# tritonmedia/beholder

Hardware: AMD Instinct MI355X
Metric: metric_events_ingested_per_sec (higher is better)
Workload: dtype protobuf-events (no tensor compute); 1 GPU; model=beholder telemetry consumer (status+progress handlers, index.js:62-155), global_batch=65536, parallelism=dp1 x 1 consumer proc/rank (BASELINE: single process per consumer)

## Files before the change

### beholder_amd/ops/csrc/py_handlers.cpp

```cpp
#include <cstdlib>
#include <string>
#include <vector>

#include "native_api.hpp"
#include "py_common.hpp"

namespace beholder {
PyTypeObject* h1_response_type();
PyObject* h1_response_status(PyObject* resp);
}
#include "gil_clock.hpp"
#include "ring.hpp"

namespace beholder {

bool text_js_str_append(std::string& out, PyObject* v);
bool text_query_pair_append(std::string& out, PyObject* k, PyObject* v, bool* first, bool rfc3986);
PyObject* pg_pool_execute_c(PyObject* nets, PyObject* sql, PyObject* params, PyObject* spread_at, PyObject* size);
PyObject* h1_call_new(PyObject* client, PyObject* method, PyObject* url, PyObject* params, PyObject* timeout,
                      bool front);
bool is_native_logger(PyObject* logger);
bool logcore_emit(PyObject* logger, bool native, long lvl, PyObject* const* args, Py_ssize_t nargs);
bool sink_stats_record(PyObject* stats, PyObject* status, double seconds);
bool is_sink_stats(PyObject* o);
// ... 248 lines not shown
bool catch_and_warn(HandlersObject* hs, PyObject* text) {
  if (!PyErr_ExceptionMatches(PyExc_Exception)) return false;
  PyObject *et, *ev, *tb;
  PyErr_Fetch(&et, &ev, &tb);
  PyErr_NormalizeException(&et, &ev, &tb);
  Py_XDECREF(tb);
  Py_XDECREF(et);
  if (ev) PyException_SetTraceback(ev, Py_None);
  PyObject* msg = PyObject_CallOneArg(hs->err_message, ev ? ev : Py_None);
  Py_XDECREF(ev);
  if (!msg) return false;
  PyObject* args[2] = {text, msg};
  bool ok = log_line(hs, 40, args, 2);
  Py_DECREF(msg);
  return ok;
}

PySendResult finish_ack(CallObject* c, PyObject** result) {
  c->done = 1;
  PyObject* r = Py_TYPE(c->rmsg) == &DeliveryType ? delivery_ack_c(c->rmsg)
                                                   : PyObject_CallMethodNoArgs(c->rmsg, s_ack);
  if (!r) return PYGEN_ERROR;
  *result = r;
  return PYGEN_RETURN;
}

PySendResult fail(CallObject* c) {
  c->done = 1;
  return PYGEN_ERROR;
}

bool raise_to_lower_case(HandlersObject* hs) {
  PyErr_SetObject(hs->js_type_error, hs->x[X_ERR_TO_LOWER]);
  return false;
}

PyObject* const* const kStoreKeys[3] = {&s_pool, &s_select, &s_update};
PyObject* const* const kPoolKeys[4] = {&s_native_pick, &s_conns, &s_spread_at, &s_size};

int pg_execute(CallObject* c, PyObject* store, PyObject* sql_name, PyObject* params, PyObject** out) {
  HandlersObject* hs = c->hs;
  if (reinterpret_cast<PyObject*>(Py_TYPE(store)) != hs->pg_cls) return 2;
  PyObject** dp = _PyObject_GetDictPtr(store);
  PyObject* sd = dp ? *dp : nullptr;
  if (!sd || !PyDict_CheckExact(sd)) return 2;
  if (!hs->store_view.refresh(sd, kStoreKeys)) return -1;
  PyObject* pool = hs->store_view.v[0];
  PyObject* sql = sql_name == s_select ? hs->store_view.v[1] : sql_name == s_update ? hs->store_view.v[2] : nullptr;
  if (!sql && pool && sql_name != s_select && sql_name != s_update) {
    sql = PyDict_GetItemWithError(sd, sql_name);
    if (!sql && PyErr_Occurred()) return -1;
  }
  if (!pool || pool == Py_None || !sql) return 2;
  PyObject** pdp = reinterpret_cast<PyObject*>(Py_TYPE(pool)) == hs->pool_cls ? _PyObject_GetDictPtr(pool) : nullptr;
  PyObject* pd = pdp ? *pdp : nullptr;
  if (pd && PyDict_CheckExact(pd) && !hs->pool_view.refresh(pd, kPoolKeys)) return -1;
  PyObject* pick = pd && PyDict_CheckExact(pd) ? hs->pool_view.v[0] : nullptr;
  if (pick && pick == hs->pick_fn) {
    PyObject* conns = hs->pool_view.v[1];
    PyObject* spread = hs->pool_view.v[2];
    PyObject* size = hs->pool_view.v[3];
    if (conns && spread && size && PyList_CheckExact(conns)) {
      Py_INCREF(conns);
      PyObject* f = pg_pool_execute_c(conns, sql, params, spread, size);
      Py_DECREF(conns);
      if (!f) return -1;
      if (f != Py_None) return await_start(c, f, out);
      Py_DECREF(f);
    }
  }
  PyObject* args[3] = {pool, sql, params};
  Py_INCREF(pool);
  PyObject* aw = PyObject_VectorcallMethod(s_execute, args, 3, nullptr);
  Py_DECREF(pool);
  if (!aw) return -1;
  return await_start(c, aw, out);
}

void untrack_row(PyObject* t) {
  if (!PyObject_GC_IsTracked(t) || Py_TYPE(t)->tp_dictoffset != 0) return;
  for (Py_ssize_t i = 0, n = PyTuple_GET_SIZE(t); i < n; ++i) {
    PyObject* v = PyTuple_GET_ITEM(t, i);
    if (PyObject_IS_GC(v) && PyObject_GC_IsTracked(v)) return;
  }
  PyObject_GC_UnTrack(t);
}

PyObject* pg_media(CallObject* c, PyObject* res) {
  HandlersObject* hs = c->hs;
  PyObject* rows = PyTuple_Check(res) && PyTuple_GET_SIZE(res) == 2 ? PyTuple_GET_ITEM(res, 0) : nullptr;
  if (!rows || !PyList_Check(rows)) {
    Py_DECREF(res);
    PyErr_SetString(PyExc_TypeError, "unexpected Postgres result");
    return nullptr;
  }
  if (PyList_GET_SIZE(rows) == 0) {
    Py_DECREF(res);
    PyErr_SetObject(hs->not_found, c->media_id);
    return nullptr;
  }
  PyObject* r = PyList_GET_ITEM(rows, 0);
  Py_INCREF(r);
  Py_DECREF(res);
  bool fast = hs->media_cls && PyTuple_CheckExact(r) && PyTuple_GET_SIZE(r) == 10;
  for (Py_ssize_t i = 0; fast && i < 10; ++i) {
    PyObject* v = PyTuple_GET_ITEM(r, i);
    bool is_int_col = i == 2 || i == 4 || i == 5 || i == 7 || i == 9;
    if (v == Py_None || (is_int_col && !PyLong_CheckExact(v))) fast = false;
  }
  PyObject* m;
  if (fast) {
    PyObject* args = PyTuple_Pack(1, r);
    m = args ? PyTuple_Type.tp_new(reinterpret_cast<PyTypeObject*>(hs->media_cls), args, nullptr) : nullptr;
    Py_XDECREF(args);
    if (m) untrack_row(m);
  } else {
    m = PyObject_CallOneArg(hs->row_to_media, r);
  }
  Py_DECREF(r);
  return m;
}

}

void untrack_atomic_row(PyObject* t) { untrack_row(t); }

namespace {

int get_media(CallObject* c, PyObject** out) {
  HandlersObject* hs = c->hs;
  PyObject* store = hattr(hs, s_store);
  if (!store) return -1;
  if (reinterpret_cast<PyObject*>(Py_TYPE(store)) == hs->memory_cls) {
    PyObject** dp = _PyObject_GetDictPtr(store);
    PyObject* sd = dp ? *dp : nullptr;
    PyObject* rows = sd ? PyDict_GetItemWithError(sd, s_rows) : nullptr;
    PyObject* calls = rows ? PyDict_GetItemWithError(sd, s_get_calls) : nullptr;
    if (calls && PyDict_CheckExact(rows)) {
      PyObject* n = PyNumber_Add(calls, hs->one);
      if (!n) return -1;
      int rc = PyDict_SetItem(sd, s_get_calls, n);
      Py_DECREF(n);
      if (rc < 0) return -1;
      PyObject* m = PyDict_GetItemWithError(rows, c->media_id);
      if (!m) {
        if (!PyErr_Occurred()) PyErr_SetObject(hs->not_found, c->media_id);
        return -1;
      }
      Py_INCREF(m);
      *out = m;
      return 1;
    }
    if (PyErr_Occurred()) return -1;
  }
  PyObject* params = PyTuple_Pack(1, c->media_id);
  if (!params) return -1;
  int k = pg_execute(c, store, s_select, params, out);
  Py_DECREF(params);
  if (k != 2) {
    if (k == 0) c->pg_get = 1;
    if (k == 1 && !(*out = pg_media(c, *out))) return -1;
    return k;
  }
  PyObject* get = hattr(hs, s_get_nowait);
  if (!get) return -1;
  if (get != Py_None) {
    PyObject* m = PyObject_CallOneArg(get, c->media_id);
    if (!m) return -1;
    *out = m;
    return 1;
  }
  PyObject* aw = PyObject_CallMethodOneArg(store, s_get_by_id, c->media_id);
  if (!aw) return -1;
  return await_start(c, aw, out);
}

int update_inline(CallObject* c) {
  HandlersObject* hs = c->hs;
  PyObject* store = hattr(hs, s_store);
  if (!store) return -1;
  if (reinterpret_cast<PyObject*>(Py_TYPE(store)) != hs->memory_cls || !hs->media_cls ||
      !PyLong_CheckExact(c->status))
    return 0;
  PyObject** dp = _PyObject_GetDictPtr(store);
  PyObject* sd = dp ? *dp : nullptr;
  PyObject* rows = sd ? PyDict_GetItemWithError(sd, s_rows) : nullptr;
  PyObject* calls = rows ? PyDict_GetItemWithError(sd, s_update_calls) : nullptr;
  if (!calls || !PyDict_CheckExact(rows)) return PyErr_Occurred() ? -1 : 0;
  PyObject* n = PyNumber_Add(calls, hs->one);
  if (!n) return -1;
  int rc = PyDict_SetItem(sd, s_update_calls, n);
  Py_DECREF(n);
  if (rc < 0) return -1;
  PyObject* m = PyDict_GetItemWithError(rows, c->media_id);
  if (!m) return PyErr_Occurred() ? -1 : 1;
  if (reinterpret_cast<PyObject*>(Py_TYPE(m)) != hs->media_cls) {
    PyObject* kw = Py_BuildValue("{s:O}", "status", c->status);
    PyObject* meth = kw ? PyObject_GetAttrString(m, "_replace") : nullptr;
    PyObject* nm = meth ? PyObject_Call(meth, PyTuple_New(0), kw) : nullptr;
    Py_XDECREF(meth);
    Py_XDECREF(kw);
    if (!nm) return -1;
    rc = PyDict_SetItem(rows, c->media_id, nm);
    Py_DECREF(nm);
    return rc < 0 ? -1 : 1;
  }
  Py_ssize_t len = PyTuple_GET_SIZE(m);
  PyObject* items = PyTuple_New(len);
  if (!items) return -1;
  for (Py_ssize_t i = 0; i < len; ++i) {
    PyObject* v = i == hs->ix_m[2] ? c->status : PyTuple_GET_ITEM(m, i);
    Py_INCREF(v);
    PyTuple_SET_ITEM(items, i, v);
  }
  PyObject* args = PyTuple_Pack(1, items);
  Py_DECREF(items);
  if (!args) return -1;
  PyObject* nm = PyTuple_Type.tp_new(reinterpret_cast<PyTypeObject*>(hs->media_cls), args, nullptr);
  Py_DECREF(args);
  if (!nm) return -1;
  untrack_row(nm);
  rc = PyDict_SetItem(rows, c->media_id, nm);
  Py_DECREF(nm);
  return rc < 0 ? -1 : 1;
}

bool record_stats(PyObject* stats, PyObject* status, double seconds) {
  if (is_sink_stats(stats)) return sink_stats_record(stats, status, seconds);
  PyObject* sec = PyFloat_FromDouble(seconds);
  if (!sec) return false;
  PyObject* r = PyObject_CallMethodObjArgs(stats, s_record, status, sec, nullptr);
  Py_DECREF(sec);
  if (!r) return false;
  Py_DECREF(r);
  return true;
}

void count_request(CallObject* c) {
  if (c->nreq < 255) ++c->nreq;
}

PyObject* const* const kHttpKeys[2] = {&s_native_record, &s_native_call};

PyObject* http_request(CallObject* c, PyObject* http, PyObject* method, PyObject* url, PyObject* params,
                       PyObject* timeout) {
  HandlersObject* hs = c->hs;
  const bool front = c->nreq > 0;
  count_request(c);
  PyObject** dp = _PyObject_GetDictPtr(http);
  PyObject* hd = dp && *dp && PyDict_CheckExact(*dp) ? *dp : nullptr;
  if (hd && !hs->http_view.refresh(hd, kHttpKeys)) return nullptr;
  PyObject* rec = hd ? hs->http_view.v[0] : nullptr;
  if (rec && PyCapsule_CheckExact(rec) && PyCapsule_IsValid(rec, kSinkHookName)) {
    const SinkHook* hook = static_cast<const SinkHook*>(PyCapsule_GetPointer(rec, kSinkHookName));
    PyObject* self = static_cast<PyObject*>(PyCapsule_GetContext(rec));
    if (!hook || !self || hook->abi != kSinkHookAbi) {
      if (!PyErr_Occurred()) PyErr_SetString(PyExc_RuntimeError, "native_record: incompatible sink hook");
      return nullptr;
    }
    Py_INCREF(rec);
    PyObject* r = hook->request(self, method, url, params ? params : Py_None);
    Py_DECREF(rec);
    return r;
  }
  PyObject* cur = hd ? hs->http_view.v[1] : nullptr;
  if (cur && cur == hs->h1_fast_fn) {
    PyObject* call = h1_call_new(http, method, url, params ? params : Py_None, timeout, front);
    if (call != Py_None) return call;
    Py_DECREF(call);
  } else if (PyErr_Occurred()) {
    return nullptr;
  }
  if (params) {
    PyObject* args[5] = {http, method, url, params, timeout};
    return PyObject_VectorcallMethod(s_request, args, 3, kw_params_timeout);
  }
  PyObject* args[4] = {http, method, url, timeout};
  return PyObject_VectorcallMethod(s_request, args, 3, kw_timeout);
}

PyObject* request_finish(CallObject* c, PyObject* value) {
  if (!c->req_native) return value;
  c->req_native = 0;
  PyObject* stats = c->req_stats;
  c->req_stats = nullptr;
  double dt = double(gil_mono_ns() - c->req_t0) * 1e-9;
  if (!value) {
    if (stats) {
      PyObject *et, *ev, *tb;
      PyErr_Fetch(&et, &ev, &tb);
      if (record_stats(stats, Py_None, dt)) {
        PyErr_Restore(et, ev, tb);
      } else {
        Py_XDECREF(et);
        Py_XDECREF(ev);
        Py_XDECREF(tb);
      }
      Py_DECREF(stats);
    }
    return nullptr;
  }
  PyObject* rt = reinterpret_cast<PyObject*>(h1_response_type());
  long code = -1;
  if (rt && reinterpret_cast<PyObject*>(Py_TYPE(value)) == rt) {
    PyObject* st = h1_response_status(value);
    if (st && PyLong_CheckExact(st)) {
      code = PyLong_AsLong(st);
      if (code == -1 && PyErr_Occurred()) PyErr_Clear();
    }
  }
  if (stats) {
    PyObject* st = PyObject_GetAttr(value, s_status);
    bool ok = st && record_stats(stats, st, dt);
    Py_XDECREF(st);
    Py_DECREF(stats);
    if (!ok) {
      Py_DECREF(value);
      return nullptr;
    }
  }
  if (c->req_strict && !(code >= 200 && code < 300)) {
    PyObject* r = PyObject_CallMethodNoArgs(value, s_raise_for_status);
    if (!r) {
      Py_DECREF(value);
      return nullptr;
    }
    Py_DECREF(r);
  }
  return value;
}

enum { TV_LIMITER, TV_RETRY, TV_KEY, TV_TOKEN, TV_BASE_URL, TV_HTTP, TV_TIMEOUT, TV_STRICT, TV_STATS, TV_N };
PyObject* const* const kTrelloKeys[TV_N] = {&s_limiter, &s_retry,   &s_key,    &s_token, &s_base_url,
                                            &s_http,    &s_timeout, &s_strict, &s_stats};

int trello_request(CallObject* c, PyObject* method, PyObject* method_upper, PyObject* path, PyObject* const* keys,
                   PyObject* const* vals, int nopt, PyObject** out) {
  HandlersObject* hs = c->hs;
  PyObject* trello = hattr(hs, s_trello);
  if (!trello) return -1;
  bool fast = reinterpret_cast<PyObject*>(Py_TYPE(trello)) == hs->trello_cls;
  PyObject** dp = fast ? _PyObject_GetDictPtr(trello) : nullptr;
  PyObject* td = dp && *dp && PyDict_CheckExact(*dp) ? *dp : nullptr;
  PyObject* const* tv = hs->trello_view.v;
  if (td) {
    if (!hs->trello_view.refresh(td, kTrelloKeys)) return -1;
    PyObject* lim = tv[TV_LIMITER];
    PyObject* rty = tv[TV_RETRY];
    if ((lim && lim != Py_None) || (rty && rty != Py_None)) td = nullptr;
  }
  PyObject* query = PyDict_New();
  if (!query) return -1;
  if (td) {
    PyObject* key = tv[TV_KEY];
    PyObject* token = key ? tv[TV_TOKEN] : nullptr;
    if (!token || PyDict_SetItem(query, hs->x[X_Q_KEY], key) < 0 || PyDict_SetItem(query, hs->x[X_Q_TOKEN], token) < 0) {
      Py_DECREF(query);
      if (PyErr_Occurred()) return -1;
      td = nullptr;
      query = PyDict_New();
      if (!query) return -1;
    }
  }
  for (int i = 0; i < nopt; ++i) {
    if (PyDict_SetItem(query, keys[i], vals[i]) < 0) {
      Py_DECREF(query);
      return -1;
    }
  }
  PyObject* aw;
  if (!td) {
    PyObject* args[4] = {trello, method, path, query};
    count_request(c);
    aw = PyObject_VectorcallMethod(s_make_request, args, 4, nullptr);
    Py_DECREF(query);
    if (!aw) return -1;
    return await_start(c, aw, out);
  }
  PyObject* base = tv[TV_BASE_URL];
  PyObject* http = base ? tv[TV_HTTP] : nullptr;
  PyObject* timeout = http ? tv[TV_TIMEOUT] : nullptr;
  PyObject* strict = timeout ? tv[TV_STRICT] : nullptr;
  PyObject* stats = strict ? tv[TV_STATS] : nullptr;
  if (!stats) {
    Py_DECREF(query);
    if (!PyErr_Occurred()) PyErr_SetString(PyExc_AttributeError, "TrelloClient attributes missing");
    return -1;
  }
  PyObject* held[5] = {base, http, timeout, strict, stats};
  for (PyObject* o : held) Py_INCREF(o);
  struct Release {
    PyObject** objs;
    ~Release() {
      for (int i = 0; i < 5; ++i) Py_DECREF(objs[i]);
    }
  } release{held};
  int is_strict = PyObject_IsTrue(strict);
  if (is_strict < 0) {
    Py_DECREF(query);
    return -1;
  }
  PyObject* url = PyUnicode_Concat(base, path);
  if (!url) {
    Py_DECREF(query);
    return -1;
  }
  c->req_t0 = gil_mono_ns();
  aw = http_request(c, http, method_upper, url, query, timeout);
  Py_DECREF(url);
  Py_DECREF(query);
  c->req_native = 1;
  c->req_strict = uint8_t(is_strict);
  if (stats != Py_None) {
    Py_INCREF(stats);
    c->req_stats = stats;
  }
  int k = aw ? await_start(c, aw, out) : -1;
  if (k != 0) {
    PyObject* v = request_finish(c, k == 1 ? *out : nullptr);
    if (!v) return -1;
    *out = v;
  }
  return k;
}

PyObject* plain_client_dict(PyObject* client, PyObject* cls) {
  if (reinterpret_cast<PyObject*>(Py_TYPE(client)) != cls) return nullptr;
  PyObject** dp = _PyObject_GetDictPtr(client);
  PyObject* d = dp ? *dp : nullptr;
  if (!d) return nullptr;
  PyObject* lim = PyDict_GetItemWithError(d, s_limiter);
  PyObject* rty = PyDict_GetItemWithError(d, s_retry);
  if (PyErr_Occurred()) {
    PyErr_Clear();
    return nullptr;
  }
  if ((lim && lim != Py_None) || (rty && rty != Py_None)) return nullptr;
  return d;
}

int sink_get(CallObject* c, PyObject* cd, std::string& url, PyObject* const* keys, PyObject* const* vals, int n,
             PyObject** out) {
  ScratchStr q_buf;
  std::string& q = *q_buf;
  bool first = true;
  for (int i = 0; i < n; ++i)
    if (!text_query_pair_append(q, keys[i], vals[i], &first, true)) return -1;
  if (!q.empty()) {
    url += url.find('?') == std::string::npos ? '?' : '&';
    url += q;
  }
  PyObject* http = PyDict_GetItemWithError(cd, s_http);
  PyObject* timeout = http ? PyDict_GetItemWithError(cd, s_timeout) : nullptr;
  PyObject* stats = timeout ? PyDict_GetItemWithError(cd, s_stats) : nullptr;
  if (!stats) {
    if (!PyErr_Occurred()) PyErr_SetString(PyExc_AttributeError, "sink client attributes missing");
    return -1;
  }
  PyObject* held[3] = {http, timeout, stats};
  for (PyObject* o : held) Py_INCREF(o);
  struct Release {
    PyObject** objs;
    ~Release() {
      for (int i = 0; i < 3; ++i) Py_DECREF(objs[i]);
    }
  } release{held};
  PyObject* full = unicode_from(url);
  if (!full) return -1;
  PyObject* aw = http_request(c, http, s_GET, full, nullptr, timeout);
  Py_DECREF(full);
  c->req_t0 = gil_mono_ns();
  c->req_native = 1;
  c->req_strict = 1;
  if (stats != Py_None) {
    Py_INCREF(stats);
    c->req_stats = stats;
  }
  int k = aw ? await_start(c, aw, out) : -1;
  if (k != 0) {
    PyObject* v = request_finish(c, k == 1 ? *out : nullptr);
    if (!v) return -1;
    *out = v;
  }
  return k;
}

int hook_telegram(CallObject* c, PyObject** out) {
  HandlersObject* hs = c->hs;
  PyObject* plan = c->plan;
  int on = PyObject_IsTrue(PyTuple_GET_ITEM(plan, 0));
  if (on <= 0) return on < 0 ? -1 : 2;
  ScratchStr line_buf;
  std::string& line = *line_buf;
  if (!tpl_append(line, hs, T_LOG_TELEGRAM, c->media_id)) return -1;
  PyObject* lo = unicode_from(line);
  bool ok = lo && log_line(hs, 30, &lo, 1);
  Py_XDECREF(lo);
  if (!ok) return -1;
  PyObject* name = PyObject_GetAttr(c->media, s_name);
  PyObject* meta = name ? PyObject_GetAttr(c->media, s_metadataId) : nullptr;
  ScratchStr text_buf;
  std::string& text = *text_buf;
  ok = meta && tpl_append(text, hs, T_TELEGRAM_TEXT, name, meta);
  Py_XDECREF(name);
  Py_XDECREF(meta);
  if (!ok) return -1;
  PyObject* textobj = unicode_from(text);
  if (!textobj) return -1;
  PyObject* tok = PyObject_CallNoArgs(PyTuple_GET_ITEM(plan, 2));
  if (!tok) {
    Py_DECREF(textobj);
    return -1;
  }
  PyObject* tg = hattr(hs, s_telegram);
  PyObject* cd = tg ? plain_client_dict(tg, hs->telegram_cls) : nullptr;
  int k;
  if (!cd) {
    if (!tg) {
      Py_DECREF(textobj);
      Py_DECREF(tok);
      return -1;
    }
    PyObject* args[5] = {tg, PyTuple_GET_ITEM(plan, 1), textobj, hs->x[X_PARSE_MODE], tok};
    PyObject* kw = PyTuple_Pack(1, s_token);
    count_request(c);
    PyObject* aw = kw ? PyObject_VectorcallMethod(s_send_message, args, 4, kw) : nullptr;
    Py_XDECREF(kw);
    Py_DECREF(textobj);
    Py_DECREF(tok);
    if (!aw) return -1;
    return await_start(c, aw, out);
  }
  PyObject* base = PyDict_GetItemWithError(cd, s_base_url);
  ScratchStr url_buf;
  std::string& url = *url_buf;
  ok = base && text_js_str_append(url, base);
  ok = ok && tpl_append(url, hs, T_PATH_TELEGRAM, tok);
  Py_DECREF(tok);
  if (!ok) {
    Py_DECREF(textobj);
    if (!PyErr_Occurred()) PyErr_SetString(PyExc_AttributeError, "TelegramClient.base_url missing");
    return -1;
  }
  PyObject* keys[3] = {hs->x[X_Q_CHAT], hs->x[X_Q_TEXT], hs->x[X_Q_PARSE_MODE]};
  PyObject* vals[3] = {PyTuple_GET_ITEM(plan, 1), textobj, hs->x[X_PARSE_MODE]};
  k = sink_get(c, cd, url, keys, vals, 3, out);
  Py_DECREF(textobj);
  return k;
}

int hook_emby(CallObject* c, PyObject** out) {
  HandlersObject* hs = c->hs;
  PyObject* plan = c->plan;
  int on = PyObject_IsTrue(PyTuple_GET_ITEM(plan, 3));
  if (on <= 0) return on < 0 ? -1 : 2;
  PyObject* host = PyTuple_GET_ITEM(plan, 4);
  PyObject* key = PyTuple_GET_ITEM(plan, 5);
  ScratchStr line_buf;
  std::string& line = *line_buf;
  if (!tpl_append(line, hs, T_LOG_EMBY, host)) return -1;
  PyObject* lo = unicode_from(line);
  bool ok = lo && log_line(hs, 30, &lo, 1);
  Py_XDECREF(lo);
  if (!ok) return -1;
  PyObject* em = hattr(hs, s_emby);
  PyObject* cd = em ? plain_client_dict(em, hs->emby_cls) : nullptr;
  if (!cd) {
    if (!em) return -1;
    PyObject* args[3] = {em, host, key};
    PyObject* kw = PyTuple_Pack(2, s_host, s_api_key);
    count_request(c);
    PyObject* aw = kw ? PyObject_VectorcallMethod(s_refresh_library, args, 1, kw) : nullptr;
    Py_XDECREF(kw);
    if (!aw) return -1;
    return await_start(c, aw, out);
  }
  ScratchStr url_buf;
  std::string& url = *url_buf;
  if (!tpl_append(url, hs, T_PATH_EMBY, host)) return -1;
  PyObject* keys[1] = {hs->x[X_Q_API_KEY]};
  PyObject* vals[1] = {key};
  return sink_get(c, cd, url, keys, vals, 1, out);
}

PySendResult step_progress(CallObject* c, PyObject* value, PyObject** result) {
  HandlersObject* hs = c->hs;
  int k;
  PyObject* v = nullptr;
  switch (c->state) {
    case 0: {
      PyObject* content = content_of(c->rmsg);
      if (!content) goto catch_;
      PyObject* msg = PyObject_CallOneArg(hs->decode_p, content);
      Py_DECREF(content);
      if (!msg) goto catch_;
      c->media_id = field(msg, hs->res_p, hs->ix_p[0], s_mediaId);
      c->status = c->media_id ? field(msg, hs->res_p, hs->ix_p[1], s_status) : nullptr;
      c->progress = c->status ? field(msg, hs->res_p, hs->ix_p[2], s_progress) : nullptr;
      c->host = c->progress ? field(msg, hs->res_p, hs->ix_p[3], s_host) : nullptr;
      Py_DECREF(msg);
      if (!c->host) goto catch_;
      {
        PyObject* args[6] = {hs->x[X_LOG_PROGRESS_0], c->media_id, hs->x[X_LOG_PROGRESS_1], c->status,
                             hs->x[X_LOG_PROGRESS_2], c->progress};
        if (!log_line(hs, 30, args, 6)) goto catch_;
      }
      PyObject* plan = PyDict_GetItemWithError(hs->progress_plan, c->status);
      if (!plan) {
        if (PyErr_Occurred()) goto catch_;
        PyObject* text = PyDict_GetItemWithError(hs->names_p, c->status);
        if (!text) {
          if (!PyErr_Occurred()) raise_to_lower_case(hs);
          goto catch_;
        }
        PyObject* lower = PyObject_CallMethodNoArgs(text, s_lower);
// ... 917 lines not shown
```

### beholder_amd/ops/csrc/py_http.cpp

```cpp
#include <cstring>
#include <string>

#include "py_common.hpp"

namespace beholder {

namespace {

enum class St : uint8_t { IDLE, HEAD, BODY_LEN, CHUNK_SIZE, CHUNK_DATA, CHUNK_CRLF, TRAILERS, BODY_EOF, DONE };

struct H1ParserObject {
  PyObject_HEAD std::string* buf;
  std::string* body;
  size_t pos;
  size_t scan;
  uint64_t remain;
  uint64_t max_header, max_body;
  int status;
  std::string* reason;
  std::string* headers;
  St st;
  bool head_req;
  bool keep_alive;
  bool http11;
  uint64_t responses;
  PyObject* last_reason;
  PyObject* last_headers;
  PyObject* last_body;
};

PyTypeObject H1ParserType = {PyVarObject_HEAD_INIT(nullptr, 0)};

inline bool is_tchar(unsigned char c) {
  return (c >= 'a' && c <= 'z') || (c >= 'A' && c <= 'Z') || (c >= '0' && c <= '9') ||
         std::strchr("!#$%&'*+-.^_`|~", c) != nullptr;
}

inline unsigned char lower(unsigned char c) { return (c >= 'A' && c <= 'Z') ? c + 32 : c; }

bool ieq(const char* a, size_t n, const char* lit) {
  size_t m = std::strlen(lit);
  if (n != m) return false;
  for (size_t i = 0; i < n; ++i)
    if (lower(static_cast<unsigned char>(a[i])) != static_cast<unsigned char>(lit[i])) return false;
  return true;
}

void trim(const char*& p, size_t& n) {
  while (n && (*p == ' ' || *p == '\t')) ++p, --n;
  while (n && (p[n - 1] == ' ' || p[n - 1] == '\t')) --n;
}

bool has_token(const char* p, size_t n, const char* token) {
  size_t i = 0;
  while (i <= n) {
    size_t j = i;
    while (j < n && p[j] != ',') ++j;
    const char* t = p + i;
    size_t tn = j - i;
    trim(t, tn);
    if (ieq(t, tn, token)) return true;
    i = j + 1;
  }
  return false;
}

bool last_is_chunked(const char* p, size_t n) {
  size_t j = n;
  while (j && p[j - 1] != ',') --j;
  const char* t = p + j;
  size_t tn = n - j;
  trim(t, tn);
  return ieq(t, tn, "chunked");
}

void reset_response(H1ParserObject* s) {
  s->status = 0;
  s->reason->clear();
  s->headers->clear();
  s->body->clear();
  s->remain = 0;
  s->keep_alive = false;
  s->http11 = false;
}

[[noreturn]] void fail(const char* what) { throw std::invalid_argument(what); }

bool next_line(const std::string& b, size_t* at, const char** p, size_t* n) {
  size_t e = b.find('\n', *at);
  if (e == std::string::npos) return false;
  *p = b.data() + *at;
  *n = e - *at;
  if (*n && (*p)[*n - 1] == '\r') --*n;
  *at = e + 1;
  return true;
}

bool parse_head(H1ParserObject* s, size_t end) {
  const std::string& b = *s->buf;
  size_t at = s->pos;
  const char* p = nullptr;
  size_t n = 0;
  if (!next_line(b, &at, &p, &n)) fail("malformed HTTP status line");
  if (n < 12 || std::memcmp(p, "HTTP/", 5) != 0 || p[5] < '0' || p[5] > '9' || p[6] != '.' || p[7] < '0' ||
      p[7] > '9' || p[8] != ' ')
    fail("malformed HTTP status line");
  int major = p[5] - '0', minor = p[7] - '0';
  if (major != 1) fail("unsupported HTTP version");
  for (int i = 9; i < 12; ++i)
    if (p[i] < '0' || p[i] > '9') fail("malformed HTTP status code");
  int status = (p[9] - '0') * 100 + (p[10] - '0') * 10 + (p[11] - '0');
  if (status < 100) fail("malformed HTTP status code");
  if (n > 12 && p[12] != ' ') fail("malformed HTTP status line");
  if (status < 200) {
    if (status == 101) fail("unexpected 101 Switching Protocols");
    s->pos = end;
    return false;
  }
  s->status = status;
  s->http11 = minor >= 1;
  if (n > 13) s->reason->assign(p + 13, n - 13);

  bool conn_close = false, conn_keep = false, chunked = false, has_te = false, has_cl = false;
  uint64_t cl = 0;
  while (at < end) {
    if (!next_line(b, &at, &p, &n) || n == 0) break;
    if (*p == ' ' || *p == '\t') fail("obsolete header line folding");
    const char* colon = static_cast<const char*>(std::memchr(p, ':', n));
    if (!colon || colon == p) fail("malformed HTTP header");
    size_t nn = size_t(colon - p);
    for (size_t i = 0; i < nn; ++i)
      if (!is_tchar(static_cast<unsigned char>(p[i]))) fail("invalid character in header name");
    const char* v = colon + 1;
    size_t vn = n - nn - 1;
    trim(v, vn);
    s->headers->append(p, n);
    s->headers->append("\r\n", 2);
    if (ieq(p, nn, "content-length")) {
      if (vn == 0 || vn > 18) fail("invalid Content-Length");
      uint64_t x = 0;
      for (size_t i = 0; i < vn; ++i) {
        if (v[i] < '0' || v[i] > '9') fail("invalid Content-Length");
        x = x * 10 + uint64_t(v[i] - '0');
      }
      if (has_cl && x != cl) fail("conflicting Content-Length headers");
      has_cl = true;
      cl = x;
    } else if (ieq(p, nn, "transfer-encoding")) {
      has_te = true;
      chunked = last_is_chunked(v, vn);
    } else if (ieq(p, nn, "connection")) {
      if (has_token(v, vn, "close")) conn_close = true;
      if (has_token(v, vn, "keep-alive")) conn_keep = true;
    }
  }
  s->pos = end;
  s->keep_alive = s->http11 ? !conn_close : (conn_keep && !conn_close);
  if (s->head_req || status == 204 || status == 304) {
    s->st = St::DONE;
  } else if (has_te) {
    if (chunked) {
      s->st = St::CHUNK_SIZE;
    } else {
      s->st = St::BODY_EOF;
      s->keep_alive = false;
    }
  } else if (has_cl) {
    if (cl > s->max_body) fail("response body exceeds max_body");
    s->remain = cl;
    s->st = cl ? St::BODY_LEN : St::DONE;
  } else {
    s->st = St::BODY_EOF;
    s->keep_alive = false;
  }
  return true;
}

void take_body(H1ParserObject* s, uint64_t want) {
  size_t avail = s->buf->size() - s->pos;
  size_t k = size_t(want < avail ? want : avail);
  s->body->append(s->buf->data() + s->pos, k);
  s->pos += k;
  s->remain -= k;
}

bool run(H1ParserObject* s) {
  std::string& b = *s->buf;
  for (;;) {
    switch (s->st) {
      case St::IDLE:
        if (s->pos < b.size()) fail("unexpected data before request");
        return false;
      case St::HEAD: {
        size_t i = s->scan > s->pos ? s->scan : s->pos;
        size_t end = std::string::npos;
        while (true) {
          size_t e = b.find('\n', i);
          if (e == std::string::npos) break;
          size_t nx = e + 1;
          if (nx < b.size() && b[nx] == '\n') {
            end = nx + 1;
            break;
          }
          if (nx + 1 < b.size() && b[nx] == '\r' && b[nx + 1] == '\n') {
            end = nx + 2;
            break;
          }
          if (nx >= b.size() || (b[nx] == '\r' && nx + 1 >= b.size())) {
            i = e;
            break;
          }
          i = nx;
        }
        if (end == std::string::npos) {
          if (b.size() - s->pos > s->max_header) fail("response header block too large");
          s->scan = i;
          return false;
        }
        if (end - s->pos > s->max_header + 4) fail("response header block too large");
        s->scan = 0;
        if (!parse_head(s, end)) continue;
        break;
      }
      case St::BODY_LEN:
        take_body(s, s->remain);
        if (s->remain) return false;
        s->st = St::DONE;
        break;
      case St::CHUNK_SIZE: {
        size_t at = s->pos;
        const char* p;
        size_t n;
        if (!next_line(b, &at, &p, &n)) {
          if (b.size() - s->pos > 4096) fail("chunk size line too long");
          return false;
        }
        size_t k = 0;
        uint64_t x = 0;
        while (k < n) {
          char c = p[k];
          int d = (c >= '0' && c <= '9') ? c - '0' : (c >= 'a' && c <= 'f') ? c - 'a' + 10
                                                   : (c >= 'A' && c <= 'F') ? c - 'A' + 10 : -1;
          if (d < 0) break;
          if (k >= 15) fail("chunk size too large");
          x = x * 16 + uint64_t(d);
          ++k;
        }
        if (k == 0) fail("malformed chunk size");
        while (k < n && (p[k] == ' ' || p[k] == '\t')) ++k;
        if (k < n && p[k] != ';') fail("malformed chunk size");
        s->pos = at;
        if (x == 0) {
          s->st = St::TRAILERS;
        } else {
          if (s->body->size() + x > s->max_body) fail("response body exceeds max_body");
          s->remain = x;
          s->st = St::CHUNK_DATA;
        }
        break;
      }
      case St::CHUNK_DATA:
        take_body(s, s->remain);
        if (s->remain) return false;
        s->st = St::CHUNK_CRLF;
        break;
      case St::CHUNK_CRLF: {
        size_t at = s->pos;
        const char* p;
        size_t n;
        if (!next_line(b, &at, &p, &n)) {
          if (b.size() - s->pos >= 2) fail("missing CRLF after chunk data");
          return false;
        }
        if (n != 0) fail("missing CRLF after chunk data");
        s->pos = at;
        s->st = St::CHUNK_SIZE;
        break;
      }
      case St::TRAILERS: {
        size_t at = s->pos;
        const char* p;
        size_t n;
        for (;;) {
          if (!next_line(b, &at, &p, &n)) {
            if (b.size() - s->pos > s->max_header) fail("trailer block too large");
            return false;
          }
          s->pos = at;
          if (n == 0) break;
        }
        s->st = St::DONE;
        break;
      }
      case St::BODY_EOF: {
        size_t avail = b.size() - s->pos;
        if (s->body->size() + avail > s->max_body) fail("response body exceeds max_body");
        s->body->append(b.data() + s->pos, avail);
        s->pos += avail;
        return false;
      }
      case St::DONE:
        return true;
    }
  }
}

PyObject* reuse_or_make(PyObject** cache, const std::string& v, bool text) {
  PyObject* c = *cache;
  if (c) {
    const char* d;
    Py_ssize_t n;
    if (text) {
      d = reinterpret_cast<const char*>(PyUnicode_1BYTE_DATA(c));
      n = PyUnicode_GET_LENGTH(c);
    } else {
      d = PyBytes_AS_STRING(c);
      n = PyBytes_GET_SIZE(c);
    }
    if (size_t(n) == v.size() && memcmp(d, v.data(), v.size()) == 0) return Py_NewRef(c);
  }
  PyObject* o;
  if (text) {
    o = PyUnicode_DecodeUTF8(v.data(), Py_ssize_t(v.size()), nullptr);
    if (!o) {
      PyErr_Clear();
      o = PyUnicode_DecodeLatin1(v.data(), Py_ssize_t(v.size()), nullptr);
    }
    if (o && !PyUnicode_IS_ASCII(o)) return o;
  } else {
    o = PyBytes_FromStringAndSize(v.data(), Py_ssize_t(v.size()));
  }
  if (!o) return nullptr;
  if (v.size() <= 4096) Py_XSETREF(*cache, Py_NewRef(o));
  return o;
}

PyObject* make_result(H1ParserObject* s) {
  PyObject* st = PyLong_FromLong(s->status);
  PyObject* reason = st ? reuse_or_make(&s->last_reason, *s->reason, true) : nullptr;
  PyObject* hdr = reason ? reuse_or_make(&s->last_headers, *s->headers, false) : nullptr;
  PyObject* body = hdr ? reuse_or_make(&s->last_body, *s->body, false) : nullptr;
  PyObject* r = body ? PyTuple_New(5) : nullptr;
  if (!r) {
    Py_XDECREF(st);
    Py_XDECREF(reason);
    Py_XDECREF(hdr);
    Py_XDECREF(body);
    return nullptr;
  }
  PyTuple_SET_ITEM(r, 0, st);
  PyTuple_SET_ITEM(r, 1, reason);
  PyTuple_SET_ITEM(r, 2, hdr);
  PyTuple_SET_ITEM(r, 3, body);
  PyTuple_SET_ITEM(r, 4, Py_NewRef(s->keep_alive ? Py_True : Py_False));
  ++s->responses;
  s->st = St::IDLE;
  s->body->clear();
  if (s->pos == s->buf->size()) {
    s->buf->clear();
    s->pos = 0;
  }
  return r;
}

void compact(H1ParserObject* s) {
  if (s->pos && (s->pos == s->buf->size() || s->pos > (s->buf->size() >> 1))) {
    s->buf->erase(0, s->pos);
    if (s->scan >= s->pos) s->scan -= s->pos; else s->scan = 0;
    s->pos = 0;
  }
}

PyObject* h1_new(PyTypeObject* type, PyObject*, PyObject*) {
  H1ParserObject* s = reinterpret_cast<H1ParserObject*>(type->tp_alloc(type, 0));
  if (!s) return nullptr;
  try {
    s->buf = new std::string();
    s->body = new std::string();
    s->reason = new std::string();
    s->headers = new std::string();
  } catch (const std::bad_alloc&) {
    Py_DECREF(s);
    return PyErr_NoMemory();
  }
  s->pos = s->scan = 0;
  s->remain = 0;
  s->max_header = 65536;
  s->max_body = 64ull << 20;
  s->st = St::IDLE;
  s->head_req = false;
  s->responses = 0;
  reset_response(s);
  return reinterpret_cast<PyObject*>(s);
}

int h1_init(H1ParserObject* s, PyObject* args, PyObject* kwds) {
  static const char* kwlist[] = {"max_header", "max_body", nullptr};
  unsigned long long mh = 65536, mb = 64ull << 20;
  if (!PyArg_ParseTupleAndKeywords(args, kwds, "|KK", const_cast<char**>(kwlist), &mh, &mb)) return -1;
  if (mh < 64) {
    PyErr_SetString(PyExc_ValueError, "max_header must be >= 64");
    return -1;
  }
  s->max_header = mh;
  s->max_body = mb;
  return 0;
}

void h1_dealloc(H1ParserObject* s) {
  Py_XDECREF(s->last_reason);
  Py_XDECREF(s->last_headers);
  Py_XDECREF(s->last_body);
  delete s->buf;
  delete s->body;
  delete s->reason;
  delete s->headers;
  Py_TYPE(s)->tp_free(reinterpret_cast<PyObject*>(s));
}

int start_core(H1ParserObject* s, bool head) {
  if (s->st != St::IDLE) {
    PyErr_SetString(PyExc_RuntimeError, "H1Parser.start() while a response is in progress");
    return -1;
  }
  reset_response(s);
  s->head_req = head;
  s->scan = 0;
  s->st = St::HEAD;
  return 0;
}

PyObject* h1_start(H1ParserObject* s, PyObject* const* args, Py_ssize_t nargs, PyObject* kwnames) {
  Py_ssize_t nkw = kwnames ? PyTuple_GET_SIZE(kwnames) : 0;
  PyObject* v = nullptr;
  if (nargs > 1 || nargs + nkw > 1) {
    PyErr_SetString(PyExc_TypeError, "start(head=False) takes one optional argument");
    return nullptr;
  }
  if (nargs == 1) {
    v = args[0];
  } else if (nkw == 1) {
    if (PyUnicode_CompareWithASCIIString(PyTuple_GET_ITEM(kwnames, 0), "head") != 0) {
      PyErr_Format(PyExc_TypeError, "start() got an unexpected keyword argument '%U'", PyTuple_GET_ITEM(kwnames, 0));
      return nullptr;
    }
    v = args[0];
  }
  int head = v ? PyObject_IsTrue(v) : 0;
  if (head < 0 || start_core(s, head != 0) < 0) return nullptr;
  Py_RETURN_NONE;
}

PyObject* feed_core(H1ParserObject* s, const char* data, size_t n) {
  BEHOLDER_TRY {
    s->buf->append(data, n);
    bool done;
    try {
      done = run(s);
    } catch (const std::invalid_argument& e) {
      s->st = St::IDLE;
      s->buf->clear();
      s->pos = 0;
      PyErr_SetString(PyExc_ValueError, e.what());
      return nullptr;
    }
    if (done) return make_result(s);
    compact(s);
    Py_RETURN_NONE;
  }
  BEHOLDER_CATCH(nullptr)
}

PyObject* h1_feed(H1ParserObject* s, PyObject* arg) {
  Py_buffer view;
  if (PyObject_GetBuffer(arg, &view, PyBUF_SIMPLE) < 0) return nullptr;
  PyObject* r = feed_core(s, static_cast<const char*>(view.buf), size_t(view.len));
  PyBuffer_Release(&view);
  return r;
}

PyObject* h1_eof(H1ParserObject* s, PyObject*) {
  BEHOLDER_TRY {
    if (s->st == St::IDLE) Py_RETURN_NONE;
    if (s->st == St::BODY_EOF) {
      s->st = St::DONE;
      return make_result(s);
    }
    if (s->st == St::DONE) return make_result(s);
    bool fresh = s->st == St::HEAD && s->pos == s->buf->size();
    s->st = St::IDLE;
    s->buf->clear();
    s->pos = 0;
    if (fresh) Py_RETURN_NONE;
    PyErr_SetString(PyExc_ValueError, "connection closed mid-response");
    return nullptr;
  }
  BEHOLDER_CATCH(nullptr)
}

PyObject* h1_get_buffered(H1ParserObject* s, void*) { return PyLong_FromSize_t(s->buf->size() - s->pos); }
PyObject* h1_get_responses(H1ParserObject* s, void*) { return PyLong_FromUnsignedLongLong(s->responses); }
PyObject* h1_get_idle(H1ParserObject* s, void*) { return PyBool_FromLong(s->st == St::IDLE); }
PyObject* h1_get_started(H1ParserObject* s, void*) {
  return PyBool_FromLong(s->st != St::IDLE && !(s->st == St::HEAD && s->pos == s->buf->size()));
}

PyMethodDef h1_methods[] = {
    {"start", reinterpret_cast<PyCFunction>(reinterpret_cast<void (*)(void)>(h1_start)), METH_FASTCALL | METH_KEYWORDS,
     "start(head=False): expect the response to a new request"},
    {"feed", reinterpret_cast<PyCFunction>(h1_feed), METH_O,
     "feed(data) -> None | (status, reason, raw_headers, body, keep_alive)"},
    {"eof", reinterpret_cast<PyCFunction>(h1_eof), METH_NOARGS,
     "eof() -> None | result: the peer closed the connection"},
    {nullptr, nullptr, 0, nullptr}};

PyGetSetDef h1_getset[] = {
    {"buffered", reinterpret_cast<getter>(h1_get_buffered), nullptr, "unconsumed input bytes", nullptr},
    {"responses", reinterpret_cast<getter>(h1_get_responses), nullptr, "complete responses parsed", nullptr},
    {"idle", reinterpret_cast<getter>(h1_get_idle), nullptr, "no response expected", nullptr},
    {"started", reinterpret_cast<getter>(h1_get_started), nullptr, "bytes of the current response seen", nullptr},
    {nullptr, nullptr, nullptr, nullptr, nullptr}};

}

bool is_h1_parser(PyObject* o) { return Py_TYPE(o) == &H1ParserType; }

int h1_parser_start_c(PyObject* o, bool head) { return start_core(reinterpret_cast<H1ParserObject*>(o), head); }

PyObject* h1_parser_feed_c(PyObject* o, const char* data, size_t n) {
  return feed_core(reinterpret_cast<H1ParserObject*>(o), data, n);
}

int init_http_types(PyObject* m) {
  H1ParserType.tp_name = "beholder_amd.ops._native.H1Parser";
  H1ParserType.tp_basicsize = sizeof(H1ParserObject);
  H1ParserType.tp_flags = Py_TPFLAGS_DEFAULT;
  H1ParserType.tp_doc = "H1Parser(max_header=65536, max_body=64MiB): incremental HTTP/1.1 response parser";
  H1ParserType.tp_new = h1_new;
  H1ParserType.tp_init = reinterpret_cast<initproc>(h1_init);
  H1ParserType.tp_dealloc = reinterpret_cast<destructor>(h1_dealloc);
  H1ParserType.tp_methods = h1_methods;
  H1ParserType.tp_getset = h1_getset;
  if (PyType_Ready(&H1ParserType) < 0) return -1;
  Py_INCREF(&H1ParserType);
  return PyModule_AddObject(m, "H1Parser", reinterpret_cast<PyObject*>(&H1ParserType));
}

}
```

Baseline: 1.237 million events/s.

## Parse complete HTTP responses in place without buffering, table-driven tchar check

Adds a fast path to the HTTP/1 parser. When a fresh response arrives whole in one feed with Content-Length framing, it is parsed directly from the input bytes, skipping the append to the internal buffer and the state-machine run. The tchar test becomes a constexpr lookup table, and the handler reuses the status object it already read from the response slot instead of calling getattr again. Anything unusual (chunked encoding, partial data, 1xx status, header folding) falls back to the existing parser, but the fast path is a second parser that has to stay consistent with the first in keep-alive and limit checks.

Measured after the change: 1.324 million events/s (median of 6 runs). +7.1%, better.

```diff
diff --git a/beholder_amd/ops/csrc/py_handlers.cpp b/beholder_amd/ops/csrc/py_handlers.cpp
--- a/beholder_amd/ops/csrc/py_handlers.cpp
+++ b/beholder_amd/ops/csrc/py_handlers.cpp
@@ -574,15 +574,16 @@
   }
   PyObject* rt = reinterpret_cast<PyObject*>(h1_response_type());
   long code = -1;
+  PyObject* slot_st = nullptr;
   if (rt && reinterpret_cast<PyObject*>(Py_TYPE(value)) == rt) {
-    PyObject* st = h1_response_status(value);
-    if (st && PyLong_CheckExact(st)) {
-      code = PyLong_AsLong(st);
+    slot_st = h1_response_status(value);
+    if (slot_st && PyLong_CheckExact(slot_st)) {
+      code = PyLong_AsLong(slot_st);
       if (code == -1 && PyErr_Occurred()) PyErr_Clear();
     }
   }
   if (stats) {
-    PyObject* st = PyObject_GetAttr(value, s_status);
+    PyObject* st = slot_st ? Py_NewRef(slot_st) : PyObject_GetAttr(value, s_status);
     bool ok = st && record_stats(stats, st, dt);
     Py_XDECREF(st);
     Py_DECREF(stats);
diff --git a/beholder_amd/ops/csrc/py_http.cpp b/beholder_amd/ops/csrc/py_http.cpp
--- a/beholder_amd/ops/csrc/py_http.cpp
+++ b/beholder_amd/ops/csrc/py_http.cpp
@@ -27,14 +27,24 @@
   PyObject* last_reason;
   PyObject* last_headers;
   PyObject* last_body;
+  uint64_t inplace;
 };
 
 PyTypeObject H1ParserType = {PyVarObject_HEAD_INIT(nullptr, 0)};
 
-inline bool is_tchar(unsigned char c) {
-  return (c >= 'a' && c <= 'z') || (c >= 'A' && c <= 'Z') || (c >= '0' && c <= '9') ||
-         std::strchr("!#$%&'*+-.^_`|~", c) != nullptr;
-}
+struct TcharTable {
+  bool v[256];
+  constexpr TcharTable() : v() {
+    for (int c = 'a'; c <= 'z'; ++c) v[c] = true;
+    for (int c = 'A'; c <= 'Z'; ++c) v[c] = true;
+    for (int c = '0'; c <= '9'; ++c) v[c] = true;
+    const char extra[] = "!#$%&'*+-.^_`|~";
+    for (int i = 0; extra[i]; ++i) v[static_cast<unsigned char>(extra[i])] = true;
+  }
+};
+constexpr TcharTable kTchar;
+
+inline bool is_tchar(unsigned char c) { return kTchar.v[c]; }
 
 inline unsigned char lower(unsigned char c) { return (c >= 'A' && c <= 'Z') ? c + 32 : c; }
 
@@ -305,7 +315,7 @@
   }
 }
 
-PyObject* reuse_or_make(PyObject** cache, const std::string& v, bool text) {
+PyObject* reuse_or_make(PyObject** cache, const char* v, size_t vn, bool text) {
   PyObject* c = *cache;
   if (c) {
     const char* d;
@@ -317,29 +327,29 @@
       d = PyBytes_AS_STRING(c);
       n = PyBytes_GET_SIZE(c);
     }
-    if (size_t(n) == v.size() && memcmp(d, v.data(), v.size()) == 0) return Py_NewRef(c);
+    if (size_t(n) == vn && memcmp(d, v, vn) == 0) return Py_NewRef(c);
   }
   PyObject* o;
   if (text) {
-    o = PyUnicode_DecodeUTF8(v.data(), Py_ssize_t(v.size()), nullptr);
+    o = PyUnicode_DecodeUTF8(v, Py_ssize_t(vn), nullptr);
     if (!o) {
       PyErr_Clear();
-      o = PyUnicode_DecodeLatin1(v.data(), Py_ssize_t(v.size()), nullptr);
+      o = PyUnicode_DecodeLatin1(v, Py_ssize_t(vn), nullptr);
     }
     if (o && !PyUnicode_IS_ASCII(o)) return o;
   } else {
-    o = PyBytes_FromStringAndSize(v.data(), Py_ssize_t(v.size()));
+    o = PyBytes_FromStringAndSize(v, Py_ssize_t(vn));
   }
   if (!o) return nullptr;
-  if (v.size() <= 4096) Py_XSETREF(*cache, Py_NewRef(o));
+  if (vn <= 4096) Py_XSETREF(*cache, Py_NewRef(o));
   return o;
 }
 
-PyObject* make_result(H1ParserObject* s) {
-  PyObject* st = PyLong_FromLong(s->status);
-  PyObject* reason = st ? reuse_or_make(&s->last_reason, *s->reason, true) : nullptr;
-  PyObject* hdr = reason ? reuse_or_make(&s->last_headers, *s->headers, false) : nullptr;
-  PyObject* body = hdr ? reuse_or_make(&s->last_body, *s->body, false) : nullptr;
+PyObject* reuse_or_make(PyObject** cache, const std::string& v, bool text) {
+  return reuse_or_make(cache, v.data(), v.size(), text);
+}
+
+PyObject* result_tuple(PyObject* st, PyObject* reason, PyObject* hdr, PyObject* body, bool keep_alive) {
   PyObject* r = body ? PyTuple_New(5) : nullptr;
   if (!r) {
     Py_XDECREF(st);
@@ -352,7 +362,17 @@
   PyTuple_SET_ITEM(r, 1, reason);
   PyTuple_SET_ITEM(r, 2, hdr);
   PyTuple_SET_ITEM(r, 3, body);
-  PyTuple_SET_ITEM(r, 4, Py_NewRef(s->keep_alive ? Py_True : Py_False));
+  PyTuple_SET_ITEM(r, 4, Py_NewRef(keep_alive ? Py_True : Py_False));
+  return r;
+}
+
+PyObject* make_result(H1ParserObject* s) {
+  PyObject* st = PyLong_FromLong(s->status);
+  PyObject* reason = st ? reuse_or_make(&s->last_reason, *s->reason, true) : nullptr;
+  PyObject* hdr = reason ? reuse_or_make(&s->last_headers, *s->headers, false) : nullptr;
+  PyObject* body = hdr ? reuse_or_make(&s->last_body, *s->body, false) : nullptr;
+  PyObject* r = result_tuple(st, reason, hdr, body, s->keep_alive);
+  if (!r) return nullptr;
   ++s->responses;
   s->st = St::IDLE;
   s->body->clear();
@@ -360,6 +380,80 @@
     s->buf->clear();
     s->pos = 0;
   }
+  return r;
+}
+
+PyObject* parse_inplace(H1ParserObject* s, const char* data, size_t n, bool* fallback) {
+  *fallback = true;
+  const char* const lim = data + n;
+  const char* e = static_cast<const char*>(std::memchr(data, '\n', n));
+  if (!e || e - data < 13 || e[-1] != '\r') return nullptr;
+  const char* p = data;
+  size_t ln = size_t(e - data) - 1;
+  if (std::memcmp(p, "HTTP/1.", 7) != 0 || p[7] < '0' || p[7] > '9' || p[8] != ' ') return nullptr;
+  for (int i = 9; i < 12; ++i)
+    if (p[i] < '0' || p[i] > '9') return nullptr;
+  int status = (p[9] - '0') * 100 + (p[10] - '0') * 10 + (p[11] - '0');
+  if (status < 200) return nullptr;
+  if (ln > 12 && p[12] != ' ') return nullptr;
+  const bool http11 = p[7] >= '1';
+  const char* reason = ln > 13 ? p + 13 : p + ln;
+  size_t reason_n = ln > 13 ? ln - 13 : 0;
+
+  const char* const hdr = e + 1;
+  const char* line = hdr;
+  bool conn_close = false, conn_keep = false, has_cl = false;
+  uint64_t cl = 0;
+  for (;;) {
+    e = static_cast<const char*>(std::memchr(line, '\n', size_t(lim - line)));
+    if (!e || e == line || e[-1] != '\r') return nullptr;
+    ln = size_t(e - line) - 1;
+    if (ln == 0) break;
+    if (*line == ' ' || *line == '\t') return nullptr;
+    size_t nn = 0;
+    while (nn < ln && is_tchar(static_cast<unsigned char>(line[nn]))) ++nn;
+    if (nn == 0 || nn == ln || line[nn] != ':') return nullptr;
+    const char* v = line + nn + 1;
+    size_t vn = ln - nn - 1;
+    if (nn == 14) {
+      if (ieq(line, nn, "content-length")) {
+        trim(v, vn);
+        if (has_cl || vn == 0 || vn > 18) return nullptr;
+        for (size_t i = 0; i < vn; ++i) {
+          if (v[i] < '0' || v[i] > '9') return nullptr;
+          cl = cl * 10 + uint64_t(v[i] - '0');
+        }
+        has_cl = true;
+      }
+    } else if (nn == 17) {
+      if (ieq(line, nn, "transfer-encoding")) return nullptr;
+    } else if (nn == 10) {
+      if (ieq(line, nn, "connection")) {
+        trim(v, vn);
+        if (has_token(v, vn, "close")) conn_close = true;
+        if (has_token(v, vn, "keep-alive")) conn_keep = true;
+      }
+    }
+    line = e + 1;
+  }
+  const char* const body = e + 1;
+  if (size_t(body - data) > s->max_header) return nullptr;
+  size_t body_n = size_t(lim - body);
+  if (s->head_req || status == 204 || status == 304) {
+    if (body_n) return nullptr;
+  } else {
+    if (!has_cl || cl > s->max_body || cl != body_n) return nullptr;
+  }
+  *fallback = false;
+  PyObject* st = PyLong_FromLong(status);
+  PyObject* ro = st ? reuse_or_make(&s->last_reason, reason, reason_n, true) : nullptr;
+  PyObject* ho = ro ? reuse_or_make(&s->last_headers, hdr, size_t(line - hdr), false) : nullptr;
+  PyObject* bo = ho ? reuse_or_make(&s->last_body, body, body_n, false) : nullptr;
+  PyObject* r = result_tuple(st, ro, ho, bo, http11 ? !conn_close : (conn_keep && !conn_close));
+  if (!r) return nullptr;
+  ++s->responses;
+  ++s->inplace;
+  s->st = St::IDLE;
   return r;
 }
 
@@ -390,6 +484,7 @@
   s->st = St::IDLE;
   s->head_req = false;
   s->responses = 0;
+  s->inplace = 0;
   reset_response(s);
   return reinterpret_cast<PyObject*>(s);
 }
@@ -453,6 +548,11 @@
 
 PyObject* feed_core(H1ParserObject* s, const char* data, size_t n) {
   BEHOLDER_TRY {
+    if (s->st == St::HEAD && s->buf->empty()) {
+      bool fallback;
+      PyObject* r = parse_inplace(s, data, n, &fallback);
+      if (!fallback) return r;
+    }
     s->buf->append(data, n);
     bool done;
     try {
@@ -500,6 +600,7 @@
 
 PyObject* h1_get_buffered(H1ParserObject* s, void*) { return PyLong_FromSize_t(s->buf->size() - s->pos); }
 PyObject* h1_get_responses(H1ParserObject* s, void*) { return PyLong_FromUnsignedLongLong(s->responses); }
+PyObject* h1_get_inplace(H1ParserObject* s, void*) { return PyLong_FromUnsignedLongLong(s->inplace); }
 PyObject* h1_get_idle(H1ParserObject* s, void*) { return PyBool_FromLong(s->st == St::IDLE); }
 PyObject* h1_get_started(H1ParserObject* s, void*) {
   return PyBool_FromLong(s->st != St::IDLE && !(s->st == St::HEAD && s->pos == s->buf->size()));
@@ -517,6 +618,7 @@
 PyGetSetDef h1_getset[] = {
     {"buffered", reinterpret_cast<getter>(h1_get_buffered), nullptr, "unconsumed input bytes", nullptr},
     {"responses", reinterpret_cast<getter>(h1_get_responses), nullptr, "complete responses parsed", nullptr},
+    {"inplace", reinterpret_cast<getter>(h1_get_inplace), nullptr, "responses parsed in place, without buffering", nullptr},
     {"idle", reinterpret_cast<getter>(h1_get_idle), nullptr, "no response expected", nullptr},
     {"started", reinterpret_cast<getter>(h1_get_started), nullptr, "bytes of the current response seen", nullptr},
     {nullptr, nullptr, nullptr, nullptr, nullptr}};
```
